# littlespray/StreamFlow

Measured on AMD Instinct MI355X. Metric: flow_fields_per_sec, higher is better.
Workload: dtype f16x2 / f16 mixed (activations fp16; weights fp16 in 24 of the 45 contraction / depthwise layers, hi+lo in the rest; fp32 accumulate); fp16 correlation volumes; 1 GPU; sintel_440x1024_T4_iters15; clips_per_launch=8, device_pinning=single device, flow_fields_per_clip=3, parallelism=replicas1, hip_graph=True, preset=config2_mixed, corr_volume=fp16 cells, single f16 MFMA product, fp32 accumulate, gma=flash (fused recompute, 1 MFMA product(s) per logit)

## Files before the change

streamflow_amd/csrc/gemm_bstat.hip:

```cpp
#include "weight_ring.h"

namespace {

typedef _Float16 f16x8 __attribute__((ext_vector_type(8)));
typedef _Float16 f16x4 __attribute__((ext_vector_type(4)));
typedef _Float16 f16x2 __attribute__((ext_vector_type(2)));
typedef float f32x16 __attribute__((ext_vector_type(16)));
typedef float f32x4 __attribute__((ext_vector_type(4)));
typedef unsigned int u32x4 __attribute__((ext_vector_type(4)));
typedef unsigned int u32x2 __attribute__((ext_vector_type(2)));
typedef __attribute__((address_space(3))) void* lds_ptr;
using sf::f32x2;
using sf::gelu_poly_n;
using sf::static_for;
using sf::wait_vm;

constexpr int kThreads = 256;
constexpr int BN = 128;
constexpr int TM = 2;
template <int PM> struct StageK { static constexpr int value = (PM == 1) ? 8 : 4; };
#ifndef SF_BSTAT_RING
#define SF_BSTAT_RING 3
#endif
constexpr int RING = SF_BSTAT_RING;
#ifndef SF_BSTAT_STORE_SLACK
#define SF_BSTAT_STORE_SLACK 1
#endif
constexpr int kParamRows = 1024;
constexpr int kOob = 1 << 30;

struct BsArgs {
    SfGemm g;
    int a_bytes;
    int nst;
    int msteps;
    int msplit;
    int n_main;
    int ntile;
    int e_ops;
};

struct WorkItem { int tile, part, nparts; };
__device__ __forceinline__ WorkItem work_item(const BsArgs& a) {
    const int w = blockIdx.x;
    WorkItem wi;
    if (w < a.n_main) { wi.tile = w; wi.part = 0; wi.nparts = 1; }
    else { wi.tile = a.n_main + (w - a.n_main) / a.msplit; wi.part = (w - a.n_main) % a.msplit; wi.nparts = a.msplit; }
    return wi;
}

template <int P>
__device__ __forceinline__ void wait_vm_epi(int e) {
    switch (e) {
        case 0: wait_vm<P>(); break;
        case 8: wait_vm<P + 8>(); break;
        case 16: wait_vm<P + 16>(); break;
        case 32: wait_vm<P + 32>(); break;
        case 40: wait_vm<P + 40>(); break;
        case 48: wait_vm<P + 48>(); break;
        default:
            if (e >= 56) wait_vm<(P + 56 > 63 ? 63 : P + 56)>();
            else wait_vm<P>();
            break;
    }
}

template <int NP>
__device__ __forceinline__ void gelu_erf_n(f32x2 (&x)[NP]) {
    f32x2 z[NP], z2[NP], p[NP], q[NP];
#pragma unroll
    for (int i = 0; i < NP; ++i) {
        z[i] = x[i] * sf::splat2(0.70710678118654752440f);
        z[i] = __builtin_elementwise_min(__builtin_elementwise_max(z[i], sf::splat2(-4.0f)), sf::splat2(4.0f));
        z2[i] = z[i] * z[i];
        p[i] = sf::splat2(-2.72614225801306e-10f);
        q[i] = sf::splat2(-1.45660718464996e-05f);
    }
    constexpr float cp[6] = {2.77068142495902e-08f, -2.10102402082508e-06f, -5.69250639462346e-05f, -7.34990630326855e-04f,
                             -2.95459980854025e-03f, -1.60960333262415e-02f};
    constexpr float cq[4] = {-2.13374055278905e-04f, -1.68282697438203e-03f, -7.37332916720468e-03f, -1.42647390514189e-02f};
#pragma unroll
    for (int k = 0; k < 6; ++k)
#pragma unroll
        for (int i = 0; i < NP; ++i) {
            p[i] = __builtin_elementwise_fma(p[i], z2[i], sf::splat2(cp[k]));
            if (k < 4) q[i] = __builtin_elementwise_fma(q[i], z2[i], sf::splat2(cq[k]));
        }
#pragma unroll
    for (int i = 0; i < NP; ++i) {
        f32x2 rq;
        rq[0] = __builtin_amdgcn_rcpf(q[i][0]);
        rq[1] = __builtin_amdgcn_rcpf(q[i][1]);
        const f32x2 e = (z[i] * p[i]) * rq;
        x[i] = sf::splat2(0.5f) * __builtin_elementwise_max(x[i], sf::splat2(-5.6568542f)) * (sf::splat2(1.0f) + e);
    }
}
template <bool kFast, int NP>
__device__ __forceinline__ void gelu_n(f32x2 (&x)[NP]) {
    if constexpr (kFast) gelu_poly_n<NP>(x);
    else gelu_erf_n<NP>(x);
}

template <int EPI, bool kFast, int NP>
__device__ __forceinline__ void epi_n(f32x2 (&v)[NP], const f32x2 (&r)[NP], const f32x2 (&dww)[NP], const f32x2 (&dwb)[NP], float gam) {
    if (EPI == SF_EPI_GELU) { gelu_n<kFast, NP>(v); return; }
    if (EPI == SF_EPI_RELU) {
#pragma unroll
        for (int i = 0; i < NP; ++i) v[i] = __builtin_elementwise_max(v[i], sf::splat2(0.f));
        return;
    }
    if (EPI == SF_EPI_RES || EPI == SF_EPI_RES_GELU || EPI == SF_EPI_RES_GELU_DW1) {
#pragma unroll
        for (int i = 0; i < NP; ++i) v[i] = r[i] + v[i];
        if (EPI == SF_EPI_RES) return;
        gelu_n<kFast, NP>(v);
        if (EPI == SF_EPI_RES_GELU) return;
#pragma unroll
        for (int i = 0; i < NP; ++i) v[i] = v[i] + (dww[i] * v[i] + dwb[i]);
        gelu_n<kFast, NP>(v);
        return;
    }
    if (EPI == SF_EPI_AXPY) {
#pragma unroll
        for (int i = 0; i < NP; ++i) v[i] = r[i] + sf::splat2(gam) * v[i];
    }
}

template <int NKS>
__device__ __forceinline__ void load_b_frags(const SfGemm& g, int z, int nc, int khalf, int nks_rt, f16x8 (&b)[NKS]) {
    if (g.b_layout == SF_LAYOUT_F16_KOCT) {
        const int noct = (g.K + 7) / 8;
        const int goct = g.b_group > 0 ? g.b_group / 8 : 0;
        const int64_t span = goct ? ((int64_t)((noct - 1) / goct) * g.b_group_stride * 2 + (int64_t)((noct - 1) % goct + 1) * g.ldb * 16)
                                  : (int64_t)noct * g.ldb * 16;
        const __amdgpu_buffer_rsrc_t rb = __builtin_amdgcn_make_buffer_rsrc(
            const_cast<char*>(reinterpret_cast<const char*>(g.B)) + (int64_t)z * g.strideB * 2, 0, (int)span, 0x00020000);
        const int vo = (khalf * (int)g.ldb + nc) * 16;
        int so = 0, oin = 0, gbase = 0;
        const int ostep = 2 * (int)g.ldb * 16, gstep = (int)(g.b_group_stride * 2);
#pragma unroll
        for (int ks = 0; ks < NKS; ++ks) {
            if (ks < nks_rt) {
                b[ks] = __builtin_bit_cast(f16x8, __builtin_amdgcn_raw_buffer_load_b128(rb, (2 * ks + khalf < noct) ? vo : kOob, so, 0));
                so += ostep; oin += 2;
                if (goct && oin == goct) { oin = 0; gbase += gstep; so = gbase; }
            }
        }
    } else if (g.b_layout == SF_LAYOUT_K_MAJOR) {
        const int kl = g.K - 1;
        const int64_t last = (g.b_group > 0) ? (int64_t)(kl / g.b_group) * g.b_group_stride + (int64_t)(kl % g.b_group) * g.ldb
                                             : (int64_t)kl * g.ldb;
        const __amdgpu_buffer_rsrc_t rb = __builtin_amdgcn_make_buffer_rsrc(
            const_cast<float*>(g.B) + (int64_t)z * g.strideB, 0, (int)((last + g.N) * 4), 0x00020000);
        const int vo = (khalf * 8 * (int)g.ldb + nc) * 4;
        int so = 0, kin = 0, gbase = 0;
        const int rstep = (int)g.ldb * 4, gstep = (int)(g.b_group_stride * 4);
#pragma unroll
        for (int ks = 0; ks < NKS; ++ks) {
            if (ks < nks_rt) {
                f16x8 f;
#pragma unroll
                for (int i = 0; i < 8; ++i) {
                    const unsigned u = __builtin_amdgcn_raw_buffer_load_b32(rb, (ks * 16 + i + 8 * khalf < g.K) ? vo : kOob, so + i * rstep, 0);
                    f[i] = (_Float16)__builtin_bit_cast(float, u);
                }
                b[ks] = f;
                so += 16 * rstep; kin += 16;
                if (g.b_group > 0 && kin == g.b_group) { kin = 0; gbase += gstep; so = gbase; }
            }
            if ((ks & 3) == 3) __builtin_amdgcn_sched_barrier(0);
        }
    } else {
        const __amdgpu_buffer_rsrc_t rb = __builtin_amdgcn_make_buffer_rsrc(
            const_cast<char*>(reinterpret_cast<const char*>(g.B)) + (int64_t)z * g.strideB * 2, 0,
            (int)(((int64_t)(g.K - 1) * g.ldb + g.N) * 2), 0x00020000);
        const int vo = (khalf * 8 * (int)g.ldb + nc) * 2;
        const int rstep = (int)g.ldb * 2;
#pragma unroll
        for (int ks = 0; ks < NKS; ++ks) {
            if (ks < nks_rt) {
                f16x8 f;
#pragma unroll
                for (int i = 0; i < 8; ++i) {
                    const unsigned short u = __builtin_amdgcn_raw_buffer_load_b16(rb, (ks * 16 + i + 8 * khalf < g.K) ? vo : kOob, (ks * 16 + i) * rstep, 0);
                    f[i] = __builtin_bit_cast(_Float16, u);
                }
                b[ks] = f;
            }
            if ((ks & 3) == 3) __builtin_amdgcn_sched_barrier(0);
        }
    }

}

template <int NKS, int PM, int RES>
__global__ __launch_bounds__(kThreads, (PM == 1 && NKS <= 16 && RES == 0) ? 4 : 2) void gemm_bstat_kernel(const BsArgs a) {
    const SfGemm& g = a.g;
    constexpr int SKS = StageK<PM>::value;
    constexpr int NST = NKS / SKS;
    constexpr int OCT = SKS * 2;
    constexpr int kPlane = OCT * 64 * 16;
    constexpr int kStage = PM * kPlane;
    constexpr int kPieces = kStage / 1024 / 4;
    __shared__ __attribute__((aligned(1024))) char smem[RING * kStage + 3 * kParamRows * 4];
    float* sbias = reinterpret_cast<float*>(smem + RING * kStage);
    float* sdww = sbias + kParamRows;
    float* sdwb = sdww + kParamRows;

    const int tid = threadIdx.x, lane = tid & 63;
    const int wave = __builtin_amdgcn_readfirstlane(tid >> 6);
    const int khalf = lane >> 5, l31 = lane & 31;
    const WorkItem wi = work_item(a);
    const int tile = wi.tile % a.ntile, z = wi.tile / a.ntile;
    const int n = tile * BN + wave * 32 + l31, nc = min(n, g.N - 1);
    const int ms_beg = (int)((int64_t)a.msteps * wi.part / wi.nparts), ms_end = (int)((int64_t)a.msteps * (wi.part + 1) / wi.nparts);
    const int nst = a.nst;

    f16x8 b[NKS];
    load_b_frags<NKS>(g, z, nc, khalf, nst * SKS, b);

    const __amdgpu_buffer_rsrc_t rah = __builtin_amdgcn_make_buffer_rsrc(const_cast<void*>(g.A_hi), 0, a.a_bytes, 0x00020000);
    const __amdgpu_buffer_rsrc_t ral = __builtin_amdgcn_make_buffer_rsrc(const_cast<void*>(g.A_lo), 0, a.a_bytes, 0x00020000);
    auto issue_a = [&](int m, int s, int slot) {
#pragma unroll
        for (int i = 0; i < kPieces; ++i) {
            const int idx = wave + 4 * i, p = idx / OCT, o = idx % OCT;
            const int so = ((s * OCT + o) * (int)g.lda_h + m * 64) * 16;
            char* dst = smem + slot * kStage + p * kPlane + o * 1024;
            __builtin_amdgcn_raw_ptr_buffer_load_lds((PM == 2 && p) ? ral : rah, (lds_ptr)dst, 16, lane * 16, so, 0, 0);
        }
    };
    int ma = ms_beg, sa = 0;
    auto advance = [&]() {
        const bool wrap = (sa + 1 == nst);
        sa = wrap ? 0 : sa + 1;
        ma = (wrap && ma + 1 < ms_end) ? ma + 1 : ma;
    };
#pragma unroll
    for (int i = 0; i < RING - 1; ++i) {
        issue_a(ma, sa, i);
        advance();
    }

    for (int i = tid; i < a.msteps * 64; i += kThreads) {
        const bool in = i < g.M;
        sbias[i] = (in && g.bias) ? g.bias[i] : 0.f;
        if (g.epilogue == SF_EPI_RES_GELU_DW1) {
            sdww[i] = in ? g.dw_w[i] : 0.f;
            sdwb[i] = in ? g.dw_b[i] : 0.f;
        }
    }
    const float gam = (g.epilogue == SF_EPI_AXPY) ? g.gamma[0] : 0.f;

    __amdgpu_buffer_rsrc_t rr = rah;
    if (RES == 1) {
        const int mr = g.M - 1;
        const int64_t last = (g.r_group > 0) ? (int64_t)(mr / g.r_group) * g.r_group_stride + (int64_t)(mr % g.r_group) * g.ldr
                                             : (int64_t)mr * g.ldr;
        rr = __builtin_amdgcn_make_buffer_rsrc(const_cast<float*>(g.R) + (int64_t)z * g.strideR, 0, (int)((last + g.N) * 4), 0x00020000);
    } else if (RES == 2) {
        rr = __builtin_amdgcn_make_buffer_rsrc(const_cast<char*>(reinterpret_cast<const char*>(g.R)) + (int64_t)z * g.strideR * 2, 0,
                                               (int)((int64_t)((g.M + 7) / 8) * g.ldr * 16), 0x00020000);
    }
    float rf[(RES == 1) ? TM : 1][16];
    u32x2 rk[(RES == 2) ? TM : 1][4];
    auto load_res = [&](int m) {
        if (RES == 1) {
            const int vo = (4 * khalf * (int)g.ldr + nc) * 4;
#pragma unroll
            for (int t = 0; t < TM; ++t) {
                const int row0 = m * 64 + t * 32;
                const int base = (g.r_group > 0) ? (int)(((int64_t)(row0 / g.r_group) * g.r_group_stride + (int64_t)(row0 % g.r_group) * g.ldr) * 4)
                                                 : row0 * (int)g.ldr * 4;
#pragma unroll
                for (int r = 0; r < 16; ++r) {
                    const int dr = (r & 3) + 8 * (r >> 2);
                    rf[t][r] = __builtin_bit_cast(float, __builtin_amdgcn_raw_buffer_load_b32(
                        rr, (4 * khalf < __builtin_amdgcn_readfirstlane(g.M - row0 - dr)) ? vo : kOob, base + dr * (int)g.ldr * 4, 0));
                }
            }
        } else if (RES == 2) {
#pragma unroll
            for (int t = 0; t < TM; ++t)
#pragma unroll
                for (int j = 0; j < 4; ++j) {
                    const int mr = m * 64 + t * 32 + 8 * j;
                    rk[t][j] = __builtin_amdgcn_raw_buffer_load_b64(rr, (4 * khalf < __builtin_amdgcn_readfirstlane(g.M - mr)) ? (nc * 16 + khalf * 8) : kOob,
                                                                    (mr >> 3) * (int)g.ldr * 16, 0);
                }
        }
    };

    const int ces = 4;
    const __amdgpu_buffer_rsrc_t rc32 = __builtin_amdgcn_make_buffer_rsrc(
        reinterpret_cast<char*>(g.C) + (int64_t)z * g.strideC * ces, 0, (g.c_f16 == 2) ? 0 : (int)(((int64_t)(g.M - 1) * g.ldc + g.N) * 4), 0x00020000);
    _Float16* c16 = (g.c_f16 == 2) ? reinterpret_cast<_Float16*>(g.C) + (int64_t)z * g.strideC
                                   : reinterpret_cast<_Float16*>(g.C16) + (int64_t)z * g.strideC16;
    const __amdgpu_buffer_rsrc_t rc16 = __builtin_amdgcn_make_buffer_rsrc(
        c16, 0, (g.c_f16 >= 2) ? (int)((int64_t)((g.M + 7) / 8) * g.ldc * 16) : 0, 0x00020000);

    f32x16 acc[TM];
    const int lane_c32 = (n < g.N) ? (4 * khalf * (int)g.ldc + n) * 4 : kOob;
    const int lane_k16 = (n < g.N) ? n * 16 + khalf * 8 : kOob;
    const int ldc4 = (int)g.ldc * 4;
    const int k4 = 4 * khalf;
    auto rows_left = [&](int r) { return __builtin_amdgcn_readfirstlane(g.M - r); };
    auto rows_left8 = [&](int r) { return __builtin_amdgcn_readfirstlane((g.M + 7) / 8 * 8 - r); };
    auto epilogue = [&](int m, auto epi_tag, auto cf_tag) {
        constexpr int EPI = decltype(epi_tag)::value;
        constexpr int CF = decltype(cf_tag)::value;
        constexpr bool kFast = (CF == 2);
#pragma unroll
        for (int t = 0; t < TM; ++t)
#pragma unroll
            for (int j0 = 0; j0 < 4; j0 += 2) {
                f32x2 v[4], r[4], dww[4], dwb[4];
#pragma unroll
                for (int q = 0; q < 4; ++q) {
                    const int j = j0 + (q >> 1), e = (q & 1) * 2, rb = m * 64 + t * 32 + 8 * j;
                    v[q][0] = g.alpha * acc[t][4 * j + e];
                    v[q][1] = g.alpha * acc[t][4 * j + e + 1];
                    r[q] = sf::splat2(0.f); dww[q] = sf::splat2(0.f); dwb[q] = sf::splat2(0.f);
                    if (RES == 1) { r[q][0] = rf[t][4 * j + e]; r[q][1] = rf[t][4 * j + e + 1]; }
                    if (RES == 2) {
                        const unsigned u = rk[t][j][e >> 1];
                        const f16x2 h = __builtin_bit_cast(f16x2, u);
                        r[q][0] = (float)h[0]; r[q][1] = (float)h[1];
                    }
                    if (EPI == SF_EPI_RES_GELU_DW1) {
                        dww[q] = *reinterpret_cast<const f32x2*>(sdww + rb + 4 * khalf + e);
                        dwb[q] = *reinterpret_cast<const f32x2*>(sdwb + rb + 4 * khalf + e);
                    }
                }
                epi_n<EPI, kFast, 4>(v, r, dww, dwb, gam);
#pragma unroll
                for (int jj = 0; jj < 2; ++jj) {
                    const int j = j0 + jj, rb = m * 64 + t * 32 + 8 * j;
                    const float o[4] = {v[2 * jj][0], v[2 * jj][1], v[2 * jj + 1][0], v[2 * jj + 1][1]};
                    if (CF != 2) {
#pragma unroll
                        for (int e = 0; e < 4; ++e)
                            __builtin_amdgcn_raw_buffer_store_b32(__builtin_bit_cast(unsigned, o[e]), rc32,
                                                                  (k4 < rows_left(rb + e)) ? lane_c32 : kOob, (rb + e) * ldc4, 0);
                    }
                    if (CF >= 2) {
                        f16x4 h;
#pragma unroll
                        for (int e = 0; e < 4; ++e) h[e] = (_Float16)o[e];
                        const int so = (rb >> 3) * ldc4 * 4;
                        const bool full = (CF == 2) ? (k4 < rows_left8(rb)) : (k4 < rows_left(rb + 3));
                        __builtin_amdgcn_raw_buffer_store_b64(__builtin_bit_cast(u32x2, h), rc16, full ? lane_k16 : kOob, so, 0);
                        if (CF == 3 && (g.M & 3) && rb + 8 > g.M && rb < g.M) {
#pragma unroll
                            for (int e = 0; e < 3; ++e) {
                                const _Float16 he = h[e];
                                const bool part = k4 < rows_left(rb) && !(k4 < rows_left(rb + 3)) && k4 < rows_left(rb + e);
                                __builtin_amdgcn_raw_buffer_store_b16(__builtin_bit_cast(unsigned short, he), rc16,
                                                                      part ? lane_k16 + e * 2 : kOob, so, 0);
                            }
                        }
                    }
                }
            }
    };
    auto run_cf = [&](int m, auto epi_tag) {
        using std::integral_constant;
        constexpr int EPI = decltype(epi_tag)::value;
        constexpr bool kKoctOnly = (EPI == SF_EPI_NONE || EPI == SF_EPI_GELU || EPI == SF_EPI_RES_GELU);
        if (kKoctOnly && g.c_f16 == 2) epilogue(m, epi_tag, integral_constant<int, 2>{});
        else if (g.c_f16 == 3) epilogue(m, epi_tag, integral_constant<int, 3>{});
        else epilogue(m, epi_tag, integral_constant<int, 0>{});
    };
    auto run_epilogue = [&](int m) {
        using std::integral_constant;
        switch (g.epilogue) {
            case SF_EPI_GELU: run_cf(m, integral_constant<int, SF_EPI_GELU>{}); break;
            case SF_EPI_RELU: run_cf(m, integral_constant<int, SF_EPI_RELU>{}); break;
            case SF_EPI_RES: if (RES) run_cf(m, integral_constant<int, SF_EPI_RES>{}); break;
            case SF_EPI_RES_GELU: if (RES) run_cf(m, integral_constant<int, SF_EPI_RES_GELU>{}); break;
            case SF_EPI_RES_GELU_DW1: if (RES) run_cf(m, integral_constant<int, SF_EPI_RES_GELU_DW1>{}); break;
            case SF_EPI_AXPY: if (RES) run_cf(m, integral_constant<int, SF_EPI_AXPY>{}); break;
            default: run_cf(m, integral_constant<int, SF_EPI_NONE>{}); break;
        }
    };

    wait_vm<0>();
    __syncthreads();

    int slot = 0;
    const char* sa_base = smem + (khalf * 64 + l31) * 16;
    for (int m = ms_beg; m < ms_end; ++m) {
#pragma unroll
        for (int t = 0; t < TM; ++t)
#pragma unroll
            for (int j = 0; j < 4; ++j) {
                const f32x4 b4 = *reinterpret_cast<const f32x4*>(sbias + m * 64 + t * 32 + 8 * j + 4 * khalf);
#pragma unroll
                for (int e = 0; e < 4; ++e) acc[t][4 * j + e] = b4[e];
            }
        load_res(m);
        __builtin_amdgcn_sched_barrier(0);
#pragma unroll
        for (int s = 0; s < NST; ++s) {
            if (s < nst) {
                if (s < RING - 1) wait_vm_epi<kPieces * (RING - 2)>(a.e_ops);
                else wait_vm<kPieces * (RING - 2)>();
                __builtin_amdgcn_s_barrier();
                issue_a(ma, sa, slot == 0 ? RING - 1 : slot - 1);
                advance();
                __builtin_amdgcn_sched_barrier(0);
                const char* sp = sa_base + slot * kStage;
#pragma unroll
                for (int ks = 0; ks < SKS; ++ks) {
                    f16x8 ah[TM], al[TM];
                    if (PM == 2) {
#pragma unroll
                        for (int t = 0; t < TM; ++t) al[t] = *reinterpret_cast<const f16x8*>(sp + kPlane + ks * 2048 + t * 512);
                    }
#pragma unroll
                    for (int t = 0; t < TM; ++t) ah[t] = *reinterpret_cast<const f16x8*>(sp + ks * 2048 + t * 512);
#pragma unroll
                    for (int t = 0; t < TM; ++t) {
                        if (PM == 2) acc[t] = __builtin_amdgcn_mfma_f32_32x32x16_f16(al[t], b[s * SKS + ks], acc[t], 0, 0, 0);
                    }
#pragma unroll
                    for (int t = 0; t < TM; ++t) acc[t] = __builtin_amdgcn_mfma_f32_32x32x16_f16(ah[t], b[s * SKS + ks], acc[t], 0, 0, 0);
                }
                {
                    constexpr int kMfma = SKS * PM * TM, kAhead = (NKS >= 40 ? 1 : 2) * PM * TM;
                    __builtin_amdgcn_sched_group_barrier(0x100, kAhead, 0);
#pragma unroll
                    for (int i = 0; i < kMfma; ++i) {
                        __builtin_amdgcn_sched_group_barrier(0x008, 1, 0);
                        if (i + kAhead < kMfma) __builtin_amdgcn_sched_group_barrier(0x100, 1, 0);
                    }
                }
                __builtin_amdgcn_sched_barrier(0);
                slot = (slot == RING - 1) ? 0 : slot + 1;
            }
        }
        run_epilogue(m);
    }
    wait_vm<0>();
}

template <int NF> struct StageF { static constexpr int value = (NF % 16 == 0) ? 16 : (NF % 20 == 0) ? 20 : (NF % 12 == 0) ? 12 : 8; };

template <int NKS, int PM>
__global__ __launch_bounds__(kThreads, 2) void gemm_bstat_gk_kernel(const BsArgs a) {
    const SfGemm& g = a.g;
    constexpr int NF = NKS * PM, S = StageF<NF>::value, NS = NF / S, P = S / 4;
    static_assert(NF % S == 0 && S % 4 == 0, "stage size must divide the fragments of a tile");
    constexpr int kStage = S * 1024;
    __shared__ __attribute__((aligned(1024))) char smem[RING * kStage + kParamRows * 4];
    float* sbias = reinterpret_cast<float*>(smem + RING * kStage);
    const int tid = threadIdx.x, lane = tid & 63;
    const int wave = __builtin_amdgcn_readfirstlane(tid >> 6);
    const int khalf = lane >> 5, l31 = lane & 31;
    const WorkItem wi = work_item(a);
    const int tile = wi.tile % a.ntile, z = wi.tile / a.ntile;
    const int n = tile * BN + wave * 32 + l31, nc = min(n, g.N - 1);
    const int NT = (g.M + 31) / 32;
    const int t_beg = (int)((int64_t)NT * wi.part / wi.nparts), t_end = (int)((int64_t)NT * (wi.part + 1) / wi.nparts);

    f16x8 b[NKS];
    load_b_frags<NKS>(g, z, nc, khalf, NKS, b);

    const __amdgpu_buffer_rsrc_t rah = __builtin_amdgcn_make_buffer_rsrc(const_cast<void*>(g.A_hi), 0, a.a_bytes, 0x00020000);
    const __amdgpu_buffer_rsrc_t ral = __builtin_amdgcn_make_buffer_rsrc(const_cast<void*>(g.A_lo), 0, a.a_bytes, 0x00020000);
    const int voa = ((lane >> 5) * (int)g.lda_h + (lane & 31)) * 16;
    auto issue_stage = [&](int tau, int s, int slot) {
#pragma unroll
        for (int i = 0; i < P; ++i) {
            const int fi = wave + 4 * i;
            const int f = s * S + fi, ks = f / PM, pl = f % PM;
            const int so = (2 * ks * (int)g.lda_h + tau * 32) * 16;
            __builtin_amdgcn_raw_ptr_buffer_load_lds((PM == 2 && pl == 0) ? ral : rah, (lds_ptr)(smem + (slot * S + fi) * 1024), 16,
                                                     voa + so, 0, 0, 0);
        }
    };
    int ta = t_beg, sa = 0;
    auto advance = [&]() {
        const bool wrap = (sa + 1 == NS);
        sa = wrap ? 0 : sa + 1;
        ta = (wrap && ta + 1 < t_end) ? ta + 1 : ta;
    };
#pragma unroll
    for (int i = 0; i < RING - 1; ++i) {
        issue_stage(ta, sa, i);
        advance();
    }
    for (int i = tid; i < NT * 32; i += kThreads) sbias[i] = (i < g.M && g.bias) ? g.bias[i] : 0.f;

    _Float16* c16 = reinterpret_cast<_Float16*>(g.C) + (int64_t)z * g.strideC;
    const __amdgpu_buffer_rsrc_t rc16 = __builtin_amdgcn_make_buffer_rsrc(c16, 0, (int)((int64_t)((g.M + 7) / 8) * g.ldc * 16), 0x00020000);
    const int lane_k16 = (n < g.N) ? n * 16 + khalf * 8 : kOob;
    const int k4 = 4 * khalf, ldc16 = (int)g.ldc * 16;
    auto rows_left8 = [&](int r) { return __builtin_amdgcn_readfirstlane((g.M + 7) / 8 * 8 - r); };

    auto epi_groups = [&](const f32x16& acc, int tau, auto j0_tag, auto ng_tag) {
        constexpr int J0 = decltype(j0_tag)::value, NG = decltype(ng_tag)::value;
        constexpr int CH = (NKS >= 40) ? 2 : 2 * NG;
        if constexpr (NG > 0) {
            unsigned hw[2 * NG];
#pragma unroll
            for (int c = 0; c < 2 * NG; c += CH) {
                f32x2 v[CH];
#pragma unroll
                for (int q = 0; q < CH; ++q) {
                    const int j = J0 + ((c + q) >> 1), e = ((c + q) & 1) * 2;
                    v[q][0] = g.alpha * acc[4 * j + e];
                    v[q][1] = g.alpha * acc[4 * j + e + 1];
                }
                gelu_poly_n<CH>(v);
#pragma unroll
                for (int q = 0; q < CH; ++q) {
                    f16x2 h;
                    h[0] = (_Float16)v[q][0]; h[1] = (_Float16)v[q][1];
                    hw[c + q] = __builtin_bit_cast(unsigned, h);
                }
            }
#pragma unroll
            for (int jj = 0; jj < NG; ++jj) {
// ... 42 lines not shown
            constexpr int kJ0 = s * kBase + (s < kRem ? s : kRem), kGroups = kBase + (s < kRem ? 1 : 0);
            if constexpr (kPrev) epi_groups(prev, tau - 1, integral_constant<int, kJ0>{}, integral_constant<int, kGroups>{});
            issue_stage(ta, sa, slot == 0 ? RING - 1 : slot - 1);
            advance();
            {
                constexpr int kAhead = 3;
                constexpr int kValu = kPrev ? (40 * kGroups + S - 1) / S : 0;
                __builtin_amdgcn_sched_group_barrier(0x002, 1, 0);
                __builtin_amdgcn_sched_group_barrier(0x100, kAhead, 0);
#pragma unroll
                for (int i = 0; i < S; ++i) {
                    __builtin_amdgcn_sched_group_barrier(0x008, 1, 0);
                    if (i + kAhead < S) __builtin_amdgcn_sched_group_barrier(0x100, 1, 0);
                    if (kValu > 0) __builtin_amdgcn_sched_group_barrier(0x002, kValu, 0);
                    if (i + kAhead >= S) {
                        constexpr int kPer = (P + kAhead - 1) / kAhead;
                        __builtin_amdgcn_sched_group_barrier(0x002, kPer, 0);
                        __builtin_amdgcn_sched_group_barrier(0x020, kPer, 0);
                    }
                }
            }
            __builtin_amdgcn_sched_barrier(0);
            slot = (slot == RING - 1) ? 0 : slot + 1;
        });
    };

    using std::integral_constant;
    int tau = t_beg;
    if (tau < t_end) {
        using T_ = integral_constant<bool, true>;
        using F_ = integral_constant<bool, false>;
        phase(acc0, acc1, tau, F_{}, F_{});
        ++tau;
        if (tau + 1 < t_end) {
            phase(acc1, acc0, tau, T_{}, F_{});
            phase(acc0, acc1, tau + 1, T_{}, T_{});
            tau += 2;
        }
        while (tau + 1 < t_end) {
            phase(acc1, acc0, tau, T_{}, T_{});
            phase(acc0, acc1, tau + 1, T_{}, T_{});
            tau += 2;
        }
        if (tau < t_end) {
            phase(acc1, acc0, tau, T_{}, F_{});
            epi_groups(acc1, tau, integral_constant<int, 0>{}, integral_constant<int, 2>{});
            epi_groups(acc1, tau, integral_constant<int, 2>{}, integral_constant<int, 2>{});
        } else {
            epi_groups(acc0, tau - 1, integral_constant<int, 0>{}, integral_constant<int, 2>{});
            epi_groups(acc0, tau - 1, integral_constant<int, 2>{}, integral_constant<int, 2>{});
        }
    }
    wait_vm<0>();
}

template <int PM>
int launch_gk(const BsArgs& a, dim3 grid, hipStream_t st) {
    const int nks = (a.g.K + 15) / 16;
    const bool probe = sf::gemm_route_probe() != nullptr;
    int sel;
    if (nks <= 8) { sel = 8; if (!probe) hipLaunchKernelGGL((gemm_bstat_gk_kernel<8, PM>), grid, dim3(kThreads), 0, st, a); }
    else if (nks <= 16) { sel = 16; if (!probe) hipLaunchKernelGGL((gemm_bstat_gk_kernel<16, PM>), grid, dim3(kThreads), 0, st, a); }
    else if (nks <= 24) { sel = 24; if (!probe) hipLaunchKernelGGL((gemm_bstat_gk_kernel<24, PM>), grid, dim3(kThreads), 0, st, a); }
    else if (nks <= 32) { sel = 32; if (!probe) hipLaunchKernelGGL((gemm_bstat_gk_kernel<32, PM>), grid, dim3(kThreads), 0, st, a); }
    else { sel = 40; if (!probe) hipLaunchKernelGGL((gemm_bstat_gk_kernel<40, PM>), grid, dim3(kThreads), 0, st, a); }
    if (probe) return sf::gemm_route_report(SF_GEMM_FAMILY_BSTAT_GELU, 0, PM, sel, 0, a.msplit, a.n_main);
    return sf::check_launch("sf_gemm(B-stationary, pipelined GELU)");
}

template <int NKS, int PM>
int launch_res(const BsArgs& a, dim3 grid, hipStream_t st) {
    const SfGemm& g = a.g;
    const bool needs_r = g.epilogue == SF_EPI_RES || g.epilogue == SF_EPI_RES_GELU || g.epilogue == SF_EPI_RES_GELU_DW1 ||
                         g.epilogue == SF_EPI_AXPY;
    const bool probe = sf::gemm_route_probe() != nullptr;
    int res = 0;
    if (!needs_r) { if (!probe) hipLaunchKernelGGL((gemm_bstat_kernel<NKS, PM, 0>), grid, dim3(kThreads), 0, st, a); }
    else if (g.r_f16 == 2) {
        res = 2;
        if constexpr (NKS <= 32) { if (!probe) hipLaunchKernelGGL((gemm_bstat_kernel<NKS, PM, 2>), grid, dim3(kThreads), 0, st, a); }
        else return sf::fail(SF_ERR_UNSUPPORTED, "sf_gemm(B-stationary): a k-octet residual needs K <= 512 (register budget)");
    } else {
        res = 1;
        if constexpr (NKS <= 24) { if (!probe) hipLaunchKernelGGL((gemm_bstat_kernel<NKS, PM, 1>), grid, dim3(kThreads), 0, st, a); }
        else return sf::fail(SF_ERR_UNSUPPORTED, "sf_gemm(B-stationary): an fp32 residual needs K <= 384 (register budget)");
    }
    if (probe) return sf::gemm_route_report(SF_GEMM_FAMILY_BSTAT, 0, PM, NKS, res, a.msplit, a.n_main);
    return sf::check_launch("sf_gemm(B-stationary)");
}

template <int PM>
int launch_nks(const BsArgs& a, dim3 grid, hipStream_t st) {
    const int nks = a.nst * StageK<PM>::value;
    if (nks <= 8) return launch_res<8, PM>(a, grid, st);
    if (nks <= 16) return launch_res<16, PM>(a, grid, st);
    if (nks <= 24) return launch_res<24, PM>(a, grid, st);
    if (nks <= 32) return launch_res<32, PM>(a, grid, st);
    return launch_res<40, PM>(a, grid, st);
}

}

namespace sf {

bool gemm_bstat_ok(const SfGemm& g) {
    if (g.precision != SF_PRECISION_F16X2 && g.precision != SF_PRECISION_F16) return false;
    if (g.a_layout != SF_LAYOUT_SPLIT_F16 || g.conv3x3 || g.k_splits > 1) return false;
    if (g.b_layout != SF_LAYOUT_F16_KOCT && g.b_layout != SF_LAYOUT_K_MAJOR && g.b_layout != SF_LAYOUT_F16_K_MAJOR) return false;
    if (g.K <= 64 || g.K > 640 || g.M > kParamRows || g.c_f16 == 1) return false;
    if (g.c_f16 == 2 && g.epilogue != SF_EPI_NONE && g.epilogue != SF_EPI_GELU && g.epilogue != SF_EPI_RES_GELU) return false;
    if (g.b_layout == SF_LAYOUT_F16_K_MAJOR && g.b_group) return false;
    if (g.b_group % 32 || g.r_group % 32) return false;
    if (g.a_k_pad < 128 || g.a_k_pad % 128) return false;
    const bool needs_r = g.epilogue == SF_EPI_RES || g.epilogue == SF_EPI_RES_GELU || g.epilogue == SF_EPI_RES_GELU_DW1 ||
                         g.epilogue == SF_EPI_AXPY;
    if (g.r_f16 == 2 && (!needs_r || g.r_group)) return false;
    if (needs_r && g.K > (g.r_f16 == 2 ? 512 : 384)) return false;
    if (g.c_f16 >= 2 && ((reinterpret_cast<uintptr_t>(g.c_f16 == 2 ? (void*)g.C : g.C16) & 15) || ((g.c_f16 == 2 ? g.strideC : g.strideC16) & 7) || g.ldc < g.N))
        return false;
    if (g.b_layout == SF_LAYOUT_F16_KOCT && ((reinterpret_cast<uintptr_t>(g.B) & 15) || (g.strideB & 7) || (g.b_group_stride & 7) || g.ldb < g.N))
        return false;
    if (g.r_f16 != 0 && g.r_f16 != 2) return false;
    if (needs_r && (!g.R || g.ldr < g.N)) return false;
    if (g.epilogue == SF_EPI_RES_GELU_DW1 && (!g.dw_w || !g.dw_b)) return false;
    if (g.epilogue == SF_EPI_AXPY && !g.gamma) return false;
    if (g.r_f16 == 2 && ((reinterpret_cast<uintptr_t>(g.R) & 15) || (g.strideR & 7))) return false;
    if (g.c_f16 != 2 && (!g.C || g.ldc < g.N)) return false;
    if (g.c_f16 == 3 && !g.C16) return false;
    {
        const int64_t lim = (int64_t)1 << 30;
        const int64_t noct = (g.K + 7) / 8, moct = (g.M + 7) / 8;
        int64_t bspan;
        if (g.b_layout == SF_LAYOUT_F16_KOCT)
            bspan = (g.b_group > 0 ? (int64_t)((g.K - 1) / g.b_group) * g.b_group_stride * 2 + (int64_t)((g.b_group + 7) / 8) * g.ldb * 16
                                   : noct * (int64_t)g.ldb * 16);
        else
            bspan = (g.b_group > 0 ? (int64_t)((g.K - 1) / g.b_group) * g.b_group_stride + (int64_t)(g.b_group - 1) * g.ldb + g.N
                                   : (int64_t)(g.K - 1) * g.ldb + g.N) * (g.b_layout == SF_LAYOUT_F16_K_MAJOR ? 2 : 4);
        if (bspan >= lim) return false;
        if (g.c_f16 != 2 && ((int64_t)(g.M - 1) * g.ldc + g.N) * 4 >= lim) return false;
        if (g.c_f16 >= 2 && moct * (int64_t)g.ldc * 16 >= lim) return false;
        if (needs_r) {
            const int64_t mr = g.M - 1;
            const int64_t rspan = (g.r_f16 == 2) ? moct * (int64_t)g.ldr * 16
                                : ((g.r_group > 0 ? (mr / g.r_group) * g.r_group_stride + (mr % g.r_group) * (int64_t)g.ldr : mr * (int64_t)g.ldr) + g.N) * 4;
            if (rspan >= lim) return false;
        }
    }
    return true;
}

int gemm_bstat_launch(const SfGemm& g, hipStream_t st) {
    BsArgs a{};
    a.g = g;
    const int sk = (g.precision == SF_PRECISION_F16) ? 128 : 64;
    const int kp = (g.K + 127) / 128 * 128;
    a.a_bytes = (int)((int64_t)kp * g.lda_h * 2);
    a.nst = (g.K + sk - 1) / sk;
    a.msteps = (g.M + 63) / 64;
    a.ntile = ceil_div(g.N, BN);
    const int64_t wgs = (int64_t)a.ntile * g.batch;
    const int units = (g.epilogue == SF_EPI_GELU && g.c_f16 == 2) ? (g.M + 31) / 32 : a.msteps;
    const int slots = 512;
    int n_main = (int)wgs, f = 1;
    if (wgs < slots) {
        double best = 1.0;
        for (int c = 2; c <= 4 && c <= units; ++c) {
            const double t = (double)((wgs * c + slots - 1) / slots) / c + 0.04 * (c - 1);
            if (t < best - 1e-9) { best = t; f = c; }
        }
        if (f > 1) n_main = 0;
    }
    a.n_main = n_main;
    a.msplit = f;
    {
        const bool needs_r = g.epilogue == SF_EPI_RES || g.epilogue == SF_EPI_RES_GELU || g.epilogue == SF_EPI_RES_GELU_DW1 ||
                             g.epilogue == SF_EPI_AXPY;
        a.e_ops = (g.c_f16 == 2 ? 0 : 16 * TM) + (g.c_f16 >= 2 ? 4 * TM : 0) + (!needs_r ? 0 : (g.r_f16 == 2 ? 4 * TM : 16 * TM));
        if (g.c_f16 == 3 && (g.M & 3)) a.e_ops = 0;
    }
    const int64_t grid_x = n_main + (wgs - n_main) * f;
    dim3 grid((unsigned)grid_x);
    if (g.epilogue == SF_EPI_GELU && g.c_f16 == 2) {
        return (g.precision == SF_PRECISION_F16) ? launch_gk<1>(a, grid, st) : launch_gk<2>(a, grid, st);
    }
    return (g.precision == SF_PRECISION_F16) ? launch_nks<1>(a, grid, st) : launch_nks<2>(a, grid, st);
}

}
```

streamflow_amd/csrc/gemm_split.hip:

```cpp
#include "sf_common.h"
#include "gemm_epilogue.h"
#include "split_operand.h"

namespace {

using sf::f32x16;
using sf::gemm_epilogue;

using namespace sf_split;

struct SplitArgs {
    SfGemm g;
    int64_t a_bytes, b_bytes;
};

#ifndef SF_GEMM_WAVES
#define SF_GEMM_WAVES 3
#endif
template <int WM, int WN, int TM, int TN, int ALAY, int BLAY, int PM>
__global__ __launch_bounds__(kThreads, (TM * TN >= 8) ? 2 : SF_GEMM_WAVES) void gemm_f16x3_mfma(const SplitArgs args) {
    constexpr bool SB = (PM == 3), SA = (PM >= 2);
    const SfGemm& g = args.g;
    constexpr int BM = WM * TM * 32, BN = WN * TN * 32;
    static_assert(WM * WN == 4, "4 waves per workgroup");
// ... 368 lines not shown
    }
    float* C = g.C + (int64_t)z * g.strideC + (int64_t)m * g.ldc + n;
#pragma unroll
    for (int i = 0; i < 4; ++i) {
        if (n + i < g.N) {
            const float v = g.alpha * (a[i] + bias);
            C[i] = sf::epi_apply<EPI>(v, kNeedsR ? R[i] : 0.f, dww, dwb, gam);
        }
    }
}

int launch_splitk_epilogue(const SfGemm& g, const float* part, int ks, int64_t slab, hipStream_t st) {
    dim3 grid(sf::ceil_div(sf::ceil_div(g.N, 4), 256), g.M, g.batch), block(256);
    switch (g.epilogue) {
        case SF_EPI_GELU: hipLaunchKernelGGL(splitk_epilogue_kernel<SF_EPI_GELU>, grid, block, 0, st, g, part, ks, slab); break;
        case SF_EPI_RELU: hipLaunchKernelGGL(splitk_epilogue_kernel<SF_EPI_RELU>, grid, block, 0, st, g, part, ks, slab); break;
        case SF_EPI_RES: hipLaunchKernelGGL(splitk_epilogue_kernel<SF_EPI_RES>, grid, block, 0, st, g, part, ks, slab); break;
        case SF_EPI_RES_GELU: hipLaunchKernelGGL(splitk_epilogue_kernel<SF_EPI_RES_GELU>, grid, block, 0, st, g, part, ks, slab); break;
        case SF_EPI_RES_GELU_DW1: hipLaunchKernelGGL(splitk_epilogue_kernel<SF_EPI_RES_GELU_DW1>, grid, block, 0, st, g, part, ks, slab); break;
        case SF_EPI_AXPY: hipLaunchKernelGGL(splitk_epilogue_kernel<SF_EPI_AXPY>, grid, block, 0, st, g, part, ks, slab); break;
        default: hipLaunchKernelGGL(splitk_epilogue_kernel<SF_EPI_NONE>, grid, block, 0, st, g, part, ks, slab); break;
    }
    return sf::check_launch("sf_gemm(split-K epilogue)");
}

int auto_splits(int M, int N, int K, int batch) {
    const int bm = (M > 64) ? 128 : (M > 32 ? 64 : 32);
    const long wgs = (long)((M + bm - 1) / bm) * ((N + 127) / 128) * batch;
    const int nk = (K + BK - 1) / BK;
    if (wgs >= 96 || nk < 8) return 1;
    int ks = (int)((512 + wgs - 1) / wgs);
    if (ks > nk / 3) ks = nk / 3;
    const int cap = (wgs <= 16 && nk >= 64) ? 16 : 8;
    if (ks > cap) ks = cap;
    return ks < 2 ? 1 : ks;
}

int check_output_formats(const SfGemm& g) {
    using sf::fail;
    const bool vec_c = (g.N & 3) == 0 && (g.ldc & 3) == 0 && (g.strideC & 3) == 0 && (reinterpret_cast<uintptr_t>(g.C) & 15) == 0;
    bool vec_r = true;
    if (g.R && g.r_f16 != 2)
        vec_r = (g.ldr & 3) == 0 && (g.strideR & 3) == 0 && (g.r_group_stride & 3) == 0 && (reinterpret_cast<uintptr_t>(g.R) & 15) == 0;
    if (g.c_f16 == 1 && (!vec_c || !vec_r || g.k_splits > 1))
        return fail(SF_ERR_UNSUPPORTED, "sf_gemm: c_f16 = 1 needs the vector epilogue (N, ldc, strideC, ldr, strideR %% 4 == 0, "
                                        "16-byte aligned C / R), no split-K");
    if (g.c_f16 == 3) {
        const bool ok = vec_c && vec_r && g.k_splits <= 1 && (g.strideC16 & 7) == 0 &&
                        (reinterpret_cast<uintptr_t>(g.C16) & 15) == 0 && g.ldc >= g.N;
        if (!ok)
            return fail(SF_ERR_UNSUPPORTED, "sf_gemm: c_f16 = 3 (fp32 + k-octet output) needs the vector epilogue (N, ldc, strideC, "
                                            "ldr, strideR %% 4 == 0, 16-byte aligned C / R), 16-byte aligned C16, strideC16 %% 8 == 0, "
                                            "no split-K");
    }
    if (g.c_f16 == 2 && (g.ldc < g.N || (g.strideC & 7) || (reinterpret_cast<uintptr_t>(g.C) & 15) || g.k_splits > 1 ||
                         (g.epilogue != SF_EPI_NONE && g.epilogue != SF_EPI_GELU && g.epilogue != SF_EPI_RES_GELU)))
        return fail(SF_ERR_UNSUPPORTED, "sf_gemm: c_f16 = 2 (k-octet output) needs ldc >= N, strideC %% 8 == 0, 16-byte aligned C, "
                                        "no split-K, epilogue NONE / GELU / RES_GELU");
    if (g.r_f16 != 0 && g.r_f16 != 2) return fail(SF_ERR_BAD_ARG, "sf_gemm: r_f16 must be 0 or 2");
    if (g.r_f16 == 2) {
        const bool ok = g.R && g.epilogue == SF_EPI_RES_GELU_DW1 && g.c_f16 != 2 && vec_c && g.r_group == 0 && g.ldr >= g.N &&
                        (g.strideR & 7) == 0 && (reinterpret_cast<uintptr_t>(g.R) & 15) == 0 && g.k_splits <= 1 && g.alpha != 0.f;
        if (!ok)
            return fail(SF_ERR_UNSUPPORTED, "sf_gemm: r_f16 = 2 (k-octet residual) needs epilogue RES_GELU_DW1, the vector epilogue "
                                            "(N, ldc, strideC %% 4 == 0, 16-byte aligned C), c_f16 != 2, no grouping, ldr >= N, "
                                            "16-byte aligned R, strideR %% 8 == 0, no split-K");
    }
    return SF_OK;
}

}

namespace sf {

int64_t gemm_split_ws_floats(int M, int N, int K, int batch) {
    const int ks = auto_splits(M, N, K, batch);
    return ks > 1 ? (int64_t)ks * batch * M * N : 0;
}

int gemm_split_dispatch_inner(const SfGemm& g, hipStream_t st);
bool gemm_bstat_ok(const SfGemm& g);
int gemm_bstat_launch(const SfGemm& g, hipStream_t st);

int gemm_split_dispatch(const SfGemm& g, hipStream_t st) {
    const bool to_bstat = g.algo != SF_ALGO_TILED && gemm_bstat_ok(g) &&
                          (g.algo == SF_ALGO_BSTAT || g.c_f16 == 2 || (g.b_layout == SF_LAYOUT_F16_KOCT && (g.M + 127) / 128 * 128 * 4 > g.M * 5));
    if (g.k_splits == 0 && g.split_ws && !g.conv3x3 && !g.c_f16 && !g.r_f16 && !to_bstat) {
        const int ks = auto_splits(g.M, g.N, g.K, g.batch);
        const int64_t slab = (int64_t)g.batch * g.M * g.N;
        if (ks > 1 && g.split_ws_floats >= ks * slab) {
            SfGemm p = g;
            p.C = g.split_ws; p.ldc = g.N; p.strideC = (int64_t)g.M * g.N;
            p.bias = nullptr; p.R = nullptr; p.epilogue = SF_EPI_NONE; p.alpha = 1.0f;
            p.k_splits = ks; p.split_stride = slab;
            const int rc = gemm_split_dispatch_inner(p, st);
            if (rc != SF_OK) return rc;
            if (SfGemmRoute* probe = gemm_route_probe()) { probe->k_splits = ks; return SF_OK; }
            return launch_splitk_epilogue(g, g.split_ws, ks, slab, st);
        }
    }
    return gemm_split_dispatch_inner(g, st);
}

int gemm_split_dispatch_inner(const SfGemm& g, hipStream_t st) {
    if (g.k_splits > 1 && (g.epilogue != SF_EPI_NONE || g.bias || g.k_splits > 16))
        return fail(SF_ERR_BAD_ARG, "sf_gemm(f16x3): split-K needs SF_EPI_NONE, no bias, k_splits <= 16");
    if (g.conv3x3 && (g.b_layout != SF_LAYOUT_K_MAJOR || (g.K / 9) % 32 || g.b_group || g.k_splits > 1))
        return fail(SF_ERR_UNSUPPORTED, "sf_gemm(split): conv3x3 needs a plain K-major B with Cin %% 32 == 0");
    if (g.b_group % 32) return fail(SF_ERR_BAD_ARG, "sf_gemm(f16x3): b_group must be a multiple of 32");
    SplitArgs a;
    a.g = g;
    if (g.a_layout == SF_LAYOUT_SPLIT_F16) {
        if (!g.A_hi || !g.A_lo || g.lda_h < (g.M + 127) / 128 * 128 || (g.lda_h & 127) ||
            ((reinterpret_cast<uintptr_t>(g.A_hi) | reinterpret_cast<uintptr_t>(g.A_lo)) & 15))
            return fail(SF_ERR_BAD_ARG, "sf_gemm(f16x3): SPLIT_F16 A needs 16-byte aligned A_hi/A_lo and lda_h = M padded to 128");
        if (g.a_k_pad < 0 || (g.a_k_pad & 31))
            return fail(SF_ERR_BAD_ARG, "sf_gemm(f16x3): a_k_pad must be 0 or a multiple of 32 (the k extent A_hi/A_lo are zero-padded to)");
        a.a_bytes = (int64_t)((g.K + 31) / 32 * 32) * g.lda_h * 2;
    } else {
        a.a_bytes = span_bytes(g.a_layout, g.M, g.K, g.lda, 0, 0);
    }
    a.b_bytes = span_bytes(g.b_layout, g.N, g.conv3x3 ? g.K / 9 : g.K, g.ldb, g.b_group, g.b_group_stride);
    if (a.a_bytes >= ((int64_t)1 << 31) || a.b_bytes >= ((int64_t)1 << 31))
        return fail(SF_ERR_UNSUPPORTED, "sf_gemm(f16x3): operand image larger than 2 GiB (32-bit buffer offsets)");
    const bool bstat_auto = g.c_f16 == 2 || (g.b_layout == SF_LAYOUT_F16_KOCT && (g.M + 127) / 128 * 128 * 4 > g.M * 5);
    if ((g.algo == SF_ALGO_BSTAT || (g.algo == SF_ALGO_AUTO && bstat_auto)) && gemm_bstat_ok(g)) return gemm_bstat_launch(g, st);
    if (g.algo == SF_ALGO_BSTAT) return fail(SF_ERR_UNSUPPORTED, "sf_gemm: SF_ALGO_BSTAT cannot run this problem (see include/streamflow_hip.h)");
    if (const int rc = check_output_formats(g); rc != SF_OK) return rc;
    if (g.b_layout == SF_LAYOUT_F16_KOCT) {
        if (g.a_layout != SF_LAYOUT_SPLIT_F16 || (g.precision != SF_PRECISION_F16X2 && g.precision != SF_PRECISION_F16) ||
            (g.b_group & 31) || (g.b_group_stride & 7) || g.conv3x3 || (g.strideB & 7) ||
            (reinterpret_cast<uintptr_t>(g.B) & 15) || g.ldb < g.N)
            return fail(SF_ERR_UNSUPPORTED, "sf_gemm: SF_LAYOUT_F16_KOCT B needs F16X2 / F16, a SPLIT_F16 A, groups of a multiple of "
                                            "32 rows, 16-byte aligned B, strideB and group stride, ldb >= N");
        return (g.precision == SF_PRECISION_F16) ? pick_tile<1>(a, st) : pick_tile<2>(a, st);
    }
    if (g.b_layout == SF_LAYOUT_F16_K_MAJOR) {
        if (g.a_layout != SF_LAYOUT_SPLIT_F16 || (g.precision != SF_PRECISION_F16X2 && g.precision != SF_PRECISION_F16) || (g.N & 1) || (g.ldb & 1) || (g.strideB & 1) ||
            g.b_group || g.conv3x3 || (reinterpret_cast<uintptr_t>(g.B) & 3))
            return fail(SF_ERR_UNSUPPORTED, "sf_gemm: SF_LAYOUT_F16_K_MAJOR B needs SF_PRECISION_F16X2, a SPLIT_F16 A, even N / ldb / "
                                            "strideB, no grouping, 4-byte aligned B");
        return (g.precision == SF_PRECISION_F16) ? pick_tile<1>(a, st) : pick_tile<2>(a, st);
    }
    if (g.b_layout == SF_LAYOUT_F16_K_MINOR) {
        if (g.a_layout != SF_LAYOUT_K_MINOR || (g.ldb & 1) || g.b_group || g.conv3x3 || (reinterpret_cast<uintptr_t>(g.B) & 3))
            return fail(SF_ERR_UNSUPPORTED, "sf_gemm(f16x3): SF_LAYOUT_F16_K_MINOR B needs a K-minor A, even ldb, 4-byte aligned B");
        return pick_tile<2>(a, st);
    }
    if (g.precision == SF_PRECISION_F16 && g.a_layout == SF_LAYOUT_SPLIT_F16) return pick_tile<1>(a, st);
    return (g.precision != SF_PRECISION_F16X3) ? pick_tile<2>(a, st) : pick_tile<3>(a, st);
}

}
```

Baseline: 386.9 flow-fields/s.

## Extend B-stationary GEMM to exact K tails, larger K and fp16 row output

```diff
diff --git a/streamflow_amd/csrc/gemm_bstat.hip b/streamflow_amd/csrc/gemm_bstat.hip
--- a/streamflow_amd/csrc/gemm_bstat.hip
+++ b/streamflow_amd/csrc/gemm_bstat.hip
@@ -32,6 +32,7 @@
 struct BsArgs {
     SfGemm g;
     int a_bytes;
+    int nks;
     int nst;
     int msteps;
     int msplit;
@@ -193,11 +194,16 @@
 
 }
 
+constexpr int prev_nks(int nks) { return nks <= 8 ? 0 : nks <= 16 ? 8 : nks <= 24 ? 16 : nks <= 32 ? 24 : nks <= 40 ? 32 : nks <= 48 ? 40 : 48; }
+constexpr bool one_wave(int nks, int res) { return nks > 40 || (nks > 32 && res == 1); }
+
 template <int NKS, int PM, int RES>
-__global__ __launch_bounds__(kThreads, (PM == 1 && NKS <= 16 && RES == 0) ? 4 : 2) void gemm_bstat_kernel(const BsArgs a) {
+__global__ __launch_bounds__(kThreads, one_wave(NKS, RES) ? 1 : (PM == 1 && NKS <= 16 && RES == 0) ? 4 : 2) void gemm_bstat_kernel(const BsArgs a) {
     const SfGemm& g = a.g;
     constexpr int SKS = StageK<PM>::value;
-    constexpr int NST = NKS / SKS;
+    constexpr int NST = (NKS + SKS - 1) / SKS;
+    constexpr int kPrev = prev_nks(NKS);
+    constexpr bool kShort = one_wave(NKS, RES) || (RES == 0 && NKS <= 32) || (RES == 2 && NKS <= 24);
     constexpr int OCT = SKS * 2;
     constexpr int kPlane = OCT * 64 * 16;
     constexpr int kStage = PM * kPlane;
@@ -215,9 +221,11 @@
     const int n = tile * BN + wave * 32 + l31, nc = min(n, g.N - 1);
     const int ms_beg = (int)((int64_t)a.msteps * wi.part / wi.nparts), ms_end = (int)((int64_t)a.msteps * (wi.part + 1) / wi.nparts);
     const int nst = a.nst;
+    const int nks_rt = kShort ? a.nks : nst * SKS;
+    const int nfull = nks_rt / SKS, ktail = nks_rt % SKS;
 
     f16x8 b[NKS];
-    load_b_frags<NKS>(g, z, nc, khalf, nst * SKS, b);
+    load_b_frags<NKS>(g, z, nc, khalf, nks_rt, b);
 
     const __amdgpu_buffer_rsrc_t rah = __builtin_amdgcn_make_buffer_rsrc(const_cast<void*>(g.A_hi), 0, a.a_bytes, 0x00020000);
     const __amdgpu_buffer_rsrc_t ral = __builtin_amdgcn_make_buffer_rsrc(const_cast<void*>(g.A_lo), 0, a.a_bytes, 0x00020000);
@@ -291,9 +299,10 @@
         }
     };
 
-    const int ces = 4;
+    const bool c_rows = (g.c_f16 == 1);
     const __amdgpu_buffer_rsrc_t rc32 = __builtin_amdgcn_make_buffer_rsrc(
-        reinterpret_cast<char*>(g.C) + (int64_t)z * g.strideC * ces, 0, (g.c_f16 == 2) ? 0 : (int)(((int64_t)(g.M - 1) * g.ldc + g.N) * 4), 0x00020000);
+        reinterpret_cast<char*>(g.C) + (c_rows ? (int64_t)z * g.strideC * 2 : (int64_t)z * g.strideC * 4), 0,
+        (g.c_f16 == 2) ? 0 : (c_rows ? (int)(((int64_t)(g.M - 1) * g.ldc + g.N) * 2) : (int)(((int64_t)(g.M - 1) * g.ldc + g.N) * 4)), 0x00020000);
     _Float16* c16 = (g.c_f16 == 2) ? reinterpret_cast<_Float16*>(g.C) + (int64_t)z * g.strideC
                                    : reinterpret_cast<_Float16*>(g.C16) + (int64_t)z * g.strideC16;
     const __amdgpu_buffer_rsrc_t rc16 = __builtin_amdgcn_make_buffer_rsrc(
@@ -301,8 +310,9 @@
 
     f32x16 acc[TM];
     const int lane_c32 = (n < g.N) ? (4 * khalf * (int)g.ldc + n) * 4 : kOob;
+    const int lane_r16 = (n < g.N) ? (4 * khalf * (int)g.ldc + n) * 2 : kOob;
     const int lane_k16 = (n < g.N) ? n * 16 + khalf * 8 : kOob;
-    const int ldc4 = (int)g.ldc * 4;
+    const int ldc4 = (int)g.ldc * 4, ldc2 = (int)g.ldc * 2;
     const int k4 = 4 * khalf;
     auto rows_left = [&](int r) { return __builtin_amdgcn_readfirstlane(g.M - r); };
     auto rows_left8 = [&](int r) { return __builtin_amdgcn_readfirstlane((g.M + 7) / 8 * 8 - r); };
@@ -337,7 +347,14 @@
                 for (int jj = 0; jj < 2; ++jj) {
                     const int j = j0 + jj, rb = m * 64 + t * 32 + 8 * j;
                     const float o[4] = {v[2 * jj][0], v[2 * jj][1], v[2 * jj + 1][0], v[2 * jj + 1][1]};
-                    if (CF != 2) {
+                    if (CF == 1) {
+#pragma unroll
+                        for (int e = 0; e < 4; ++e) {
+                            const _Float16 he = (_Float16)o[e];
+                            __builtin_amdgcn_raw_buffer_store_b16(__builtin_bit_cast(unsigned short, he), rc32,
+                                                                  (k4 < rows_left(rb + e)) ? lane_r16 : kOob, (rb + e) * ldc2, 0);
+                        }
+                    } else if (CF != 2) {
 #pragma unroll
                         for (int e = 0; e < 4; ++e)
                             __builtin_amdgcn_raw_buffer_store_b32(__builtin_bit_cast(unsigned, o[e]), rc32,
@@ -367,7 +384,9 @@
         using std::integral_constant;
         constexpr int EPI = decltype(epi_tag)::value;
         constexpr bool kKoctOnly = (EPI == SF_EPI_NONE || EPI == SF_EPI_GELU || EPI == SF_EPI_RES_GELU);
-        if (kKoctOnly && g.c_f16 == 2) epilogue(m, epi_tag, integral_constant<int, 2>{});
+        constexpr bool kRows = (EPI == SF_EPI_RES_GELU_DW1);
+        if (kRows && g.c_f16 == 1) epilogue(m, epi_tag, integral_constant<int, 1>{});
+        else if (kKoctOnly && g.c_f16 == 2) epilogue(m, epi_tag, integral_constant<int, 2>{});
         else if (g.c_f16 == 3) epilogue(m, epi_tag, integral_constant<int, 3>{});
         else epilogue(m, epi_tag, integral_constant<int, 0>{});
     };
@@ -400,9 +419,11 @@
             }
         load_res(m);
         __builtin_amdgcn_sched_barrier(0);
-#pragma unroll
-        for (int s = 0; s < NST; ++s) {
-            if (s < nst) {
+        static_for<0, NST>([&](auto s_tag) {
+            constexpr int s = decltype(s_tag)::value;
+            constexpr int KMAX = (NKS - s * SKS < SKS) ? NKS - s * SKS : SKS;
+            auto stage = [&](auto ks_tag) {
+                constexpr int KS = decltype(ks_tag)::value;
                 if (s < RING - 1) wait_vm_epi<kPieces * (RING - 2)>(a.e_ops);
                 else wait_vm<kPieces * (RING - 2)>();
                 __builtin_amdgcn_s_barrier();
@@ -411,7 +432,7 @@
                 __builtin_amdgcn_sched_barrier(0);
                 const char* sp = sa_base + slot * kStage;
 #pragma unroll
-                for (int ks = 0; ks < SKS; ++ks) {
+                for (int ks = 0; ks < KS; ++ks) {
                     f16x8 ah[TM], al[TM];
                     if (PM == 2) {
 #pragma unroll
@@ -427,7 +448,8 @@
                     for (int t = 0; t < TM; ++t) acc[t] = __builtin_amdgcn_mfma_f32_32x32x16_f16(ah[t], b[s * SKS + ks], acc[t], 0, 0, 0);
                 }
                 {
-                    constexpr int kMfma = SKS * PM * TM, kAhead = (NKS >= 40 ? 1 : 2) * PM * TM;
+                    constexpr int kMfma = KS * PM * TM, kWant = ((NKS >= 40 && !one_wave(NKS, RES)) ? 1 : 2) * PM * TM;
+                    constexpr int kAhead = kWant < kMfma ? kWant : kMfma;
                     __builtin_amdgcn_sched_group_barrier(0x100, kAhead, 0);
 #pragma unroll
                     for (int i = 0; i < kMfma; ++i) {
@@ -437,8 +459,17 @@
                 }
                 __builtin_amdgcn_sched_barrier(0);
                 slot = (slot == RING - 1) ? 0 : slot + 1;
-            }
-        }
+            };
+            if (s < nfull) {
+                if constexpr (KMAX == SKS) stage(std::integral_constant<int, SKS>{});
+            } else if constexpr (kShort && (s + 1) * SKS > kPrev) {
+                if (s == nfull) {
+                    static_for<1, (KMAX < SKS ? KMAX + 1 : SKS)>([&](auto ks_tag) {
+                        if (ktail == decltype(ks_tag)::value) stage(ks_tag);
+                    });
+                }
+            }
+        });
         run_epilogue(m);
     }
     wait_vm<0>();
@@ -647,8 +678,8 @@
         else return sf::fail(SF_ERR_UNSUPPORTED, "sf_gemm(B-stationary): a k-octet residual needs K <= 512 (register budget)");
     } else {
         res = 1;
-        if constexpr (NKS <= 24) { if (!probe) hipLaunchKernelGGL((gemm_bstat_kernel<NKS, PM, 1>), grid, dim3(kThreads), 0, st, a); }
-        else return sf::fail(SF_ERR_UNSUPPORTED, "sf_gemm(B-stationary): an fp32 residual needs K <= 384 (register budget)");
+        if constexpr (NKS <= 24 || NKS >= 40) { if (!probe) hipLaunchKernelGGL((gemm_bstat_kernel<NKS, PM, 1>), grid, dim3(kThreads), 0, st, a); }
+        else return sf::fail(SF_ERR_UNSUPPORTED, "sf_gemm(B-stationary): an fp32 residual needs K <= 384 or K > 512 (register budget)");
     }
     if (probe) return sf::gemm_route_report(SF_GEMM_FAMILY_BSTAT, 0, PM, NKS, res, a.msplit, a.n_main);
     return sf::check_launch("sf_gemm(B-stationary)");
@@ -656,12 +687,17 @@
 
 template <int PM>
 int launch_nks(const BsArgs& a, dim3 grid, hipStream_t st) {
-    const int nks = a.nst * StageK<PM>::value;
+    const int nks = a.nks;
     if (nks <= 8) return launch_res<8, PM>(a, grid, st);
     if (nks <= 16) return launch_res<16, PM>(a, grid, st);
     if (nks <= 24) return launch_res<24, PM>(a, grid, st);
     if (nks <= 32) return launch_res<32, PM>(a, grid, st);
-    return launch_res<40, PM>(a, grid, st);
+    if (nks <= 40) return launch_res<40, PM>(a, grid, st);
+    if constexpr (PM == 1) {
+        if (nks <= 48) return launch_res<48, 1>(a, grid, st);
+        if (nks <= 60) return launch_res<60, 1>(a, grid, st);
+    }
+    return sf::fail(SF_ERR_UNSUPPORTED, "sf_gemm(B-stationary): K beyond the built register classes");
 }
 
 }
@@ -672,7 +708,9 @@
     if (g.precision != SF_PRECISION_F16X2 && g.precision != SF_PRECISION_F16) return false;
     if (g.a_layout != SF_LAYOUT_SPLIT_F16 || g.conv3x3 || g.k_splits > 1) return false;
     if (g.b_layout != SF_LAYOUT_F16_KOCT && g.b_layout != SF_LAYOUT_K_MAJOR && g.b_layout != SF_LAYOUT_F16_K_MAJOR) return false;
-    if (g.K <= 64 || g.K > 640 || g.M > kParamRows || g.c_f16 == 1) return false;
+    if (g.K <= 64 || g.K > (g.precision == SF_PRECISION_F16 ? 960 : 640) || g.M > kParamRows) return false;
+    if (g.c_f16 == 1 && g.epilogue != SF_EPI_RES_GELU_DW1) return false;
+    if (g.K > 640 && g.epilogue == SF_EPI_GELU && g.c_f16 == 2) return false;
     if (g.c_f16 == 2 && g.epilogue != SF_EPI_NONE && g.epilogue != SF_EPI_GELU && g.epilogue != SF_EPI_RES_GELU) return false;
     if (g.b_layout == SF_LAYOUT_F16_K_MAJOR && g.b_group) return false;
     if (g.b_group % 32 || g.r_group % 32) return false;
@@ -680,7 +718,7 @@
     const bool needs_r = g.epilogue == SF_EPI_RES || g.epilogue == SF_EPI_RES_GELU || g.epilogue == SF_EPI_RES_GELU_DW1 ||
                          g.epilogue == SF_EPI_AXPY;
     if (g.r_f16 == 2 && (!needs_r || g.r_group)) return false;
-    if (needs_r && g.K > (g.r_f16 == 2 ? 512 : 384)) return false;
+    if (needs_r && (g.r_f16 == 2 ? g.K > 512 : (g.K > 384 && g.K <= 512))) return false;
     if (g.c_f16 >= 2 && ((reinterpret_cast<uintptr_t>(g.c_f16 == 2 ? (void*)g.C : g.C16) & 15) || ((g.c_f16 == 2 ? g.strideC : g.strideC16) & 7) || g.ldc < g.N))
         return false;
     if (g.b_layout == SF_LAYOUT_F16_KOCT && ((reinterpret_cast<uintptr_t>(g.B) & 15) || (g.strideB & 7) || (g.b_group_stride & 7) || g.ldb < g.N))
@@ -703,7 +741,7 @@
             bspan = (g.b_group > 0 ? (int64_t)((g.K - 1) / g.b_group) * g.b_group_stride + (int64_t)(g.b_group - 1) * g.ldb + g.N
                                    : (int64_t)(g.K - 1) * g.ldb + g.N) * (g.b_layout == SF_LAYOUT_F16_K_MAJOR ? 2 : 4);
         if (bspan >= lim) return false;
-        if (g.c_f16 != 2 && ((int64_t)(g.M - 1) * g.ldc + g.N) * 4 >= lim) return false;
+        if (g.c_f16 != 2 && ((int64_t)(g.M - 1) * g.ldc + g.N) * (g.c_f16 == 1 ? 2 : 4) >= lim) return false;
         if (g.c_f16 >= 2 && moct * (int64_t)g.ldc * 16 >= lim) return false;
         if (needs_r) {
             const int64_t mr = g.M - 1;
@@ -721,12 +759,15 @@
     const int sk = (g.precision == SF_PRECISION_F16) ? 128 : 64;
     const int kp = (g.K + 127) / 128 * 128;
     a.a_bytes = (int)((int64_t)kp * g.lda_h * 2);
+    a.nks = (g.K + 15) / 16;
     a.nst = (g.K + sk - 1) / sk;
     a.msteps = (g.M + 63) / 64;
     a.ntile = ceil_div(g.N, BN);
     const int64_t wgs = (int64_t)a.ntile * g.batch;
     const int units = (g.epilogue == SF_EPI_GELU && g.c_f16 == 2) ? (g.M + 31) / 32 : a.msteps;
-    const int slots = 512;
+    const bool fp32_r = g.r_f16 != 2 && (g.epilogue == SF_EPI_RES || g.epilogue == SF_EPI_RES_GELU || g.epilogue == SF_EPI_RES_GELU_DW1 ||
+                                         g.epilogue == SF_EPI_AXPY);
+    const int slots = one_wave(a.nks, fp32_r ? 1 : 0) ? 256 : 512;
     int n_main = (int)wgs, f = 1;
     if (wgs < slots) {
         double best = 1.0;
diff --git a/streamflow_amd/csrc/gemm_split.hip b/streamflow_amd/csrc/gemm_split.hip
--- a/streamflow_amd/csrc/gemm_split.hip
+++ b/streamflow_amd/csrc/gemm_split.hip
@@ -474,9 +474,15 @@
 bool gemm_bstat_ok(const SfGemm& g);
 int gemm_bstat_launch(const SfGemm& g, hipStream_t st);
 
+static bool gemm_bstat_auto(const SfGemm& g) {
+    const bool fp32_r = g.r_f16 == 0 && (g.epilogue == SF_EPI_RES || g.epilogue == SF_EPI_RES_GELU || g.epilogue == SF_EPI_RES_GELU_DW1 ||
+                                         g.epilogue == SF_EPI_AXPY);
+    if (g.K > 640 || (fp32_r && g.K > 512)) return false;
+    return g.c_f16 == 2 || (g.b_layout == SF_LAYOUT_F16_KOCT && (g.M + 127) / 128 * 128 * 4 > g.M * 5);
+}
+
 int gemm_split_dispatch(const SfGemm& g, hipStream_t st) {
-    const bool to_bstat = g.algo != SF_ALGO_TILED && gemm_bstat_ok(g) &&
-                          (g.algo == SF_ALGO_BSTAT || g.c_f16 == 2 || (g.b_layout == SF_LAYOUT_F16_KOCT && (g.M + 127) / 128 * 128 * 4 > g.M * 5));
+    const bool to_bstat = g.algo != SF_ALGO_TILED && gemm_bstat_ok(g) && (g.algo == SF_ALGO_BSTAT || gemm_bstat_auto(g));
     if (g.k_splits == 0 && g.split_ws && !g.conv3x3 && !g.c_f16 && !g.r_f16 && !to_bstat) {
         const int ks = auto_splits(g.M, g.N, g.K, g.batch);
         const int64_t slab = (int64_t)g.batch * g.M * g.N;
@@ -515,8 +521,7 @@
     a.b_bytes = span_bytes(g.b_layout, g.N, g.conv3x3 ? g.K / 9 : g.K, g.ldb, g.b_group, g.b_group_stride);
     if (a.a_bytes >= ((int64_t)1 << 31) || a.b_bytes >= ((int64_t)1 << 31))
         return fail(SF_ERR_UNSUPPORTED, "sf_gemm(f16x3): operand image larger than 2 GiB (32-bit buffer offsets)");
-    const bool bstat_auto = g.c_f16 == 2 || (g.b_layout == SF_LAYOUT_F16_KOCT && (g.M + 127) / 128 * 128 * 4 > g.M * 5);
-    if ((g.algo == SF_ALGO_BSTAT || (g.algo == SF_ALGO_AUTO && bstat_auto)) && gemm_bstat_ok(g)) return gemm_bstat_launch(g, st);
+    if ((g.algo == SF_ALGO_BSTAT || (g.algo == SF_ALGO_AUTO && gemm_bstat_auto(g))) && gemm_bstat_ok(g)) return gemm_bstat_launch(g, st);
     if (g.algo == SF_ALGO_BSTAT) return fail(SF_ERR_UNSUPPORTED, "sf_gemm: SF_ALGO_BSTAT cannot run this problem (see include/streamflow_hip.h)");
     if (const int rc = check_output_formats(g); rc != SF_OK) return rc;
     if (g.b_layout == SF_LAYOUT_F16_KOCT) {
```

Result: no change. 386.7 flow-fields/s (-0.1%).
